# t-mat/lz4mt

Hardware: AMD Instinct MI355X
Metric: device-resident LZ4 GiB/s (compress, decompress) on 4 MiB blocks at 1/2/4/8 MI355X (higher is better)
Workload: dtype u8

## Files before the change

lz4mt_amd/csrc/lz4mt_kernels.hip:

```cpp
#include "lz4mt_device.h"
#include <stdio.h>
#include <string.h>

#include <algorithm>
#include <atomic>
#include <mutex>

#ifndef LZ4MT_PART
#define LZ4MT_PART 0
#endif

namespace lz4mt {

[[maybe_unused]] static bool link_cold() {
    const char* e = getenv("LZ4MT_AMD_BD_COLD");
    return e && e[0] == '1';
}

static void link_stats(const char* what, const uint32_t* changed, const uint32_t* firstU, int rounds,
                       uint32_t nBlocks, hipStream_t st) {
    const char* e = getenv("LZ4MT_AMD_BD_STATS");
    if (!e || e[0] != '1') return;
    uint32_t c[kLinkRounds + 1], f[kLinkRounds + 1];
    if (hipMemcpyAsync(c, changed, sizeof(c), hipMemcpyDeviceToHost, st) != hipSuccess ||
// ... 342 lines not shown
            int w;
            uint32_t ip = 0, cd = 0, maxb = 0, lim = 0, lit0 = 0;
            bool wasTest = false, early = false, beq = false;
            uint32_t eqb = 0;
            for (;;) {
                w = sm ? __ffsll((long long)sm) - 1 : 64;
                if (w == 64 || ((tmk >> w) & 1)) break;
                ip = rdlane(p, w);
                cd = rdlane(cand, w);
                wasTest = (ballot(isTest) >> w) & 1;
                {
                    const uint32_t lowL = !LINK ? 0u : (cd >= o0 ? lk.lowIn : lk.lowDict);
                    maxb = wasTest ? 0u : min(ip - anchor, cd > lowL ? cd - lowL : 0u);
                }
                lim = matchlimit - (ip + kMinMatch);
                V.cover(min(ip + kMinMatch + 256, n));
                const bool needV = (mm >> w) & 1;
                uint32_t vx = 0;
                if (needV && L == 0) vx = ld32u(s + cd) ^ rdlane(w0, w);
                beq = false;
                if (L + 1 <= maxb) beq = V.rd1(ip - L - 1) == V.rd1(cd - L - 1);
                eqb = 0;
                if (4 * L < lim) {
                    const uint32_t x = V.rd4(ip + kMinMatch + 4 * L) ^ V.rd4(cd + kMinMatch + 4 * L);
                    eqb = x ? ((uint32_t)__builtin_ctz(x) >> 3) : 4u;
                    eqb = min(eqb, lim - 4 * L);
                }
                STAMP_ADD(3, ts);
                if (ST) acc[12] += (mm >> w) & 1;
                lit0 = ip - anchor;
                early = lit0 <= 256 && op + 1 + ext_len(lit0) + lit0 + 64 <= O.flushed + kOutRing;
                if (early) stage_lits(V, O, anchor, 0, lit0, op + 1 + ext_len(lit0), false, 0);
                STAMP_ADD(4, ts);
                if (needV && (ballot(L == 0 && vx != 0) & 1)) {
                    if (ST) acc[11] += 1;
                    sm &= ~(1ull << w);
                    STAMP_ADD(5, ts);
                    continue;
                }
                if (ST) {
                    asm volatile("s_waitcnt vmcnt(0)" ::: "memory");
                }
                STAMP_ADD(5, ts);
                break;
            }
            const bool wTerm = (w < 64) && ((tmk >> w) & 1);
            const int wlim = (w == 64) ? 63 : (wTerm ? w - 1 : w);
            if (wlim >= 0 && live && (int)L <= wlim) {
                const uint64_t later = gmask & ~mask_le(L) & mask_le((uint32_t)wlim);
                if (!later) {
                    if (U16) T16[h] = (uint16_t)p;
                    else Traw[h] = TAG ? (p | (mytag << kPosBits)) : p;
                }
            }
            WAVE_SYNC();
            STAMP_ADD(6, ts);
            if (w == 64) {
                W.k0 += 64 - ns;
                W.hasIns = 0; W.hasTest = 0;
                continue;
            }
            if (wTerm) goto last_literals;

            uint32_t back = 0, mc = 0;
            bool backDone = maxb == 0, cntDone = false;
            for (;;) {
                if (!backDone) {
                    const uint64_t fm = ballot(!beq);
                    if (fm) { back += (uint32_t)(__ffsll((long long)fm) - 1); backDone = true; }
                    else { back += 64; backDone = back >= maxb; }
                }
                if (!cntDone) {
                    const uint64_t nf = ballot(eqb < 4);
                    if (nf) {
                        const int f = __ffsll((long long)nf) - 1;
                        mc += 4 * (uint32_t)f + rdlane(eqb, f);
                        cntDone = true;
                    } else {
                        mc += 256;
                    }
                }
                if (backDone && cntDone) break;
                beq = false;
                eqb = 0;
                const uint32_t kk = back + L + 1;
                if (!backDone && kk <= maxb) beq = V.rd1(ip - kk) == V.rd1(cd - kk);
                const uint32_t rel = mc + 4 * L;
                if (!cntDone && rel < lim) {
                    const uint32_t x = V.rd4(ip + kMinMatch + rel) ^ V.rd4(cd + kMinMatch + rel);
                    eqb = x ? ((uint32_t)__builtin_ctz(x) >> 3) : 4u;
                    eqb = min(eqb, lim - rel);
                }
            }
            STAMP_ADD(7, ts);
            const uint32_t mcf = mc + back;
            const uint32_t lit = lit0 - back;
            const uint32_t litExt = ext_len(lit);
            const uint32_t mlExt = ext_len(mcf);
            if (limited) {
                if (!wasTest && op + 1 + lit + 8 + lit / 255 > cap) return 0;
                if (op + 1 + litExt + lit + 2 + 6 + (mcf + 240) / 255 > cap) return 0;
            }
            const uint32_t litPos = op + 1 + litExt;
            if (!early || litExt != ext_len(lit0)) {
                put_head(O, op, lit, mcf < 15 ? mcf : 15);
                WAVE_SYNC();
                stage_lits(V, O, anchor, 0, lit, litPos, true, litPos);
            } else {
                put_head(O, op, lit, mcf < 15 ? mcf : 15);
            }
            {
                const uint32_t off = ip - cd, tpos = litPos + lit;
                O.flush_to(tpos);
                if (L < 2) O.put(tpos + L, L == 0 ? (off & 255) : (off >> 8));
                WAVE_SYNC();
                put_ext(O, tpos + 2, mlExt, mcf >= 15 ? (mcf - 15) % 255 : 0);
            }
            op = litPos + lit + 2 + mlExt;
            WAVE_SYNC();
            O.flush_to(op);
            STAMP_ADD(8, ts);
            const uint32_t ipe = ip + kMinMatch + mc;
            anchor = ipe;
            if (ipe >= mflimitP1) goto last_literals;
            W = Win{1, 1, ipe - 2, ipe, ipe + 1, 0};
        }
    }
last_literals : {
    const uint32_t run = n - anchor;
    if (limited && op + run + 1 + (run + 240) / 255 > cap) return 0;
    put_head(O, op, run, 0);
    const uint32_t litPos = op + 1 + ext_len(run);
    WAVE_SYNC();
    stage_lits(V, O, anchor, 0, run, litPos, true, litPos);
    op = litPos + run;
    O.finish(op);
}
    return (int32_t)op;
}

typedef const __attribute__((address_space(1))) uint32_t __attribute__((aligned(1))) g_cu32u;
typedef const __attribute__((address_space(1))) uint64_t __attribute__((aligned(1))) g_cu64u;
typedef __attribute__((address_space(3))) uint64_t __attribute__((aligned(1))) l_u64u;
typedef __attribute__((address_space(3))) uint32_t __attribute__((aligned(1))) l_u32u;
typedef __attribute__((address_space(3))) uint16_t __attribute__((aligned(1))) l_u16u;
typedef __attribute__((address_space(3))) uint64_t l_u64;

constexpr uint32_t kSR = 2048;
#ifndef LZ4MT_COUNT_LANES
#define LZ4MT_COUNT_LANES 32
#endif
constexpr uint32_t kCountLanes = LZ4MT_COUNT_LANES;
#ifndef LZ4MT_CATCH_LANES
#define LZ4MT_CATCH_LANES 64
#endif
constexpr uint32_t kCatchLanes = LZ4MT_CATCH_LANES;
static_assert(kCatchLanes >= 1 && kCatchLanes <= 64, "catch-up lanes");
constexpr uint64_t kCatchMask = kCatchLanes >= 64 ? ~0ull : (1ull << kCatchLanes) - 1ull;
static_assert(kCountLanes >= 1 && kCountLanes <= 63, "count lanes");
constexpr uint32_t kSRMirror = 64;
__device__ __forceinline__ void mskor2_rtn(l_u32* w16, uint32_t m16, uint32_t d16, l_u32* w8, uint32_t m8,
                                           uint32_t d8, uint32_t& o16, uint32_t& o8) {
    asm volatile("ds_mskor_rtn_b32 %0, %2, %3, %4\n\t"
                 "ds_mskor_rtn_b32 %1, %5, %6, %7\n\t"
                 "s_waitcnt lgkmcnt(0)"
                 : "=&v"(o16), "=&v"(o8)
                 : "v"((uint32_t)(uintptr_t)w16), "v"(m16), "v"(d16), "v"((uint32_t)(uintptr_t)w8), "v"(m8), "v"(d8)
                 : "memory");
}

__device__ __forceinline__ uint32_t gld4u(g_cu8* p) { return *(g_cu32u*)p; }
__device__ __forceinline__ uint64_t gld8u(g_cu8* p) { return *(g_cu64u*)p; }

struct SrcRing {
    g_cu8* s;
    uint32_t n;
    l_u8* r;
    uint32_t B;
    uint32_t pfPos;
    uint64_t pf;

    __device__ __forceinline__ uint64_t fetch(uint32_t c) const {
        const uint32_t pos = c + 8 * laneid();
        if (pos + 8 <= n) return gld8u(s + pos);
        uint64_t v = 0;
        for (uint32_t i = 0; i < 8; ++i)
            if (pos + i < n) v |= (uint64_t)s[pos + i] << (8 * i);
        return v;
    }
    __device__ __forceinline__ void store(uint32_t c, uint64_t v) {
        const uint32_t o = (c & (kSR - 1)) + 8 * laneid();
        *(l_u64*)(r + o) = v;
        if (o < kSRMirror) *(l_u64*)(r + kSR + o) = v;
    }
    __device__ __forceinline__ void init(uint32_t b0 = 0) {
        B = b0;
        for (uint32_t c = b0; c < b0 + kSR; c += 512) store(c, fetch(c));
        pfPos = b0 + kSR;
        pf = fetch(pfPos);
        WAVE_SYNC();
    }
    __device__ __forceinline__ void cover(uint32_t hi) {
        if (hi <= B + kSR) return;
        const uint32_t nb = (hi - kSR + 511) & ~511u;
        WAVE_SYNC();
        for (uint32_t c = (nb > B + kSR ? nb : B + kSR); c < nb + kSR; c += 512) store(c, c == pfPos ? pf : fetch(c));
        B = nb;
        pfPos = B + kSR;
        pf = fetch(pfPos);
        WAVE_SYNC();
    }
    __device__ __forceinline__ uint64_t rd8(uint32_t pos) const { return *(l_u64u*)(r + (pos & (kSR - 1))); }
};

__device__ __forceinline__ uint64_t bal(bool p) { return __builtin_amdgcn_ballot_w64(p); }
__device__ __forceinline__ uint32_t sff1(uint64_t m) { return m ? (uint32_t)__builtin_ctzll(m) : 64u; }
template <bool U16, bool SPLIT = false, bool LINK = false, bool P17 = false> struct V5Geo {
    static constexpr uint32_t kTE = U16 ? 8192u : 4096u;
    static constexpr uint32_t PB = P17 ? 17u : U16 ? 16u : (LINK ? kPosBits + 1 : kPosBits);
    static constexpr uint32_t PM = (1u << PB) - 1u;
    static constexpr bool SP = SPLIT || P17;
    static constexpr uint32_t TB = P17 ? 7u : SPLIT ? 8u : 32u - PB;
    static constexpr bool HT = !SP || U16;
    static __device__ __forceinline__ uint32_t tag(uint32_t w0) {
        if constexpr (HT && U16) return ((w0 * 2654435761u) >> (19 - TB)) & ((1u << TB) - 1u);
        else if constexpr (HT) return (uint32_t)(((uint64_t)w0 << 24) * 889523592379ull >> (52 - TB)) & ((1u << TB) - 1u);
        else return (w0 * 0x85EBCA77u) >> (32 - TB);
    }
    l_u32* T;
    __device__ __forceinline__ l_u16* T16() const { return (l_u16*)T; }
    __device__ __forceinline__ l_u8* TG() const { return (l_u8*)T + 2 * (kTE + 64); }
    __device__ __forceinline__ uint32_t ld(uint32_t i) const {
        return SP ? ((uint32_t)T16()[i] | ((uint32_t)TG()[i] << 16)) : T[i];
    }
    __device__ __forceinline__ void st(uint32_t i, uint32_t e) const {
        if (SP) { T16()[i] = (uint16_t)e; TG()[i] = (uint8_t)(e >> 16); } else T[i] = e;
    }
    __device__ __forceinline__ uint32_t rb(uint32_t i) const { return SP ? (uint32_t)T16()[i] : T[i]; }
    __device__ __forceinline__ uint32_t xchg(uint32_t i, uint32_t e) const {
        if constexpr (SP) {
            const uint32_t s16 = (i & 1u) * 16u, s8 = (i & 3u) * 8u;
            uint32_t o16, o8;
            mskor2_rtn((l_u32*)T16() + (i >> 1), 0xFFFFu << s16, (e & 0xFFFFu) << s16, (l_u32*)TG() + (i >> 2),
                       0xFFu << s8, ((e >> 16) & 0xFFu) << s8, o16, o8);
            return ((o16 >> s16) & 0xFFFFu) | (((o8 >> s8) & 0xFFu) << 16);
        } else {
            return __hip_atomic_exchange(T + i, e, __ATOMIC_RELAXED, __HIP_MEMORY_SCOPE_WAVEFRONT);
        }
    }
    static constexpr uint32_t kRbMask = SP ? 0xFFFFu : 0xFFFFFFFFu;
    __device__ __forceinline__ void sweep(uint32_t Tp) const {
        const uint32_t L = laneid();
        const uint32_t mk = (Tp + 65536u) & PM;
        for (uint32_t i = L; i < kTE; i += 64) {
            const uint32_t d = (Tp - ld(i)) & PM;
            if (d > 65536u && d <= 98304u) st(i, mk);
        }
        WAVE_SYNC();
    }
    __device__ __forceinline__ void init(uint32_t e0) const {
        const uint32_t L = laneid();
        if (SP) {
            const uint32_t p2 = (e0 & 0xFFFFu) * 0x10001u, t4 = (e0 >> 16) * 0x01010101u;
            for (uint32_t i = L; i < kTE / 8; i += 64) ((l_u4*)T16())[i] = (v4u){p2, p2, p2, p2};
            for (uint32_t i = L; i < kTE / 16; i += 64) ((l_u4*)TG())[i] = (v4u){t4, t4, t4, t4};
        } else {
            for (uint32_t i = L; i < kTE / 4; i += 64) ((l_u4*)T)[i] = (v4u){e0, e0, e0, e0};
        }
    }
};

struct PendSeq {
    uint32_t op, lit, mcf, off, anchor;
    uint32_t litExt, mlExt;
};
template <bool R8> struct SeqLayout {
    uint32_t total, a1, a2, token, litRem, mlRem, off;
    __device__ __forceinline__ explicit SeqLayout(const PendSeq& e) {
        a1 = 1 + e.litExt;
        a2 = a1 + e.lit;
        total = a2 + 2 + e.mlExt;
        token = ((e.lit < 15 ? e.lit : 15) << 4) | (e.mcf < 15 ? e.mcf : 15);
        if (R8) {
            litRem = e.lit + 240 + e.litExt;
            mlRem = e.mcf + 240 + e.mlExt;
        } else {
            litRem = e.lit + 240 - __umul24(255u, e.litExt);
            mlRem = e.mcf + 240 - __umul24(255u, e.mlExt);
        }
        off = e.off;
    }
};
template <bool R8>
__device__ __forceinline__ uint32_t pend_byte(const SeqLayout<R8>& e, uint32_t x, uint32_t litByte) {
    const uint32_t vM = x + 1 < e.total ? 255u : e.mlRem;
    const uint32_t vL = x + 1 < e.a1 ? 255u : e.litRem;
    const uint32_t vO = x == e.a2 ? e.off & 255u : e.off >> 8;
    uint32_t v = x < e.a2 + 2 ? vO : vM;
    v = x < e.a2 ? litByte : v;
    v = x < e.a1 ? vL : v;
    asm volatile("" : "+v"(v));
    return x == 0 ? e.token : v;
}
template <bool R8>
__device__ __forceinline__ void store_pend(const PendSeq& p, const SrcRing& V, g_cu8* __restrict__ s,
                                           g_u8* __restrict__ d) {
    const uint32_t L = laneid();
    PendSeq q = p;
    asm volatile("" : "+v"(q.lit), "+v"(q.mcf), "+v"(q.off), "+v"(q.litExt), "+v"(q.mlExt));
    const SeqLayout<R8> e(q);
    const uint32_t total = (uint32_t)__builtin_amdgcn_readfirstlane((int)e.total);
    if (p.anchor >= V.B && p.anchor + p.lit <= V.B + kSR) {
        uint32_t base = 0;
        do {
            const uint32_t x = min(base + L, e.total - 1);
            uint32_t lv = V.r[(p.anchor + x - e.a1) & (kSR - 1)];
            asm volatile("" : "+v"(lv));
            d[p.op + x] = (uint8_t)pend_byte(e, x, lv);
            base += 64;
        } while (base < total);
    } else {
        uint32_t base = 0;
        do {
            const uint32_t x = min(base + L, e.total - 1);
            uint32_t lv = s[(x >= e.a1 && x < e.a2) ? p.anchor + x - e.a1 : p.anchor];
            asm volatile("" : "+v"(lv));
            d[p.op + x] = (uint8_t)pend_byte(e, x, lv);
            base += 64;
        } while (base < total);
    }
}

constexpr uint32_t kPubShift = 16;
[[maybe_unused]] constexpr uint32_t kPubDone = 0x80000000u, kPubRaw = 0x40000000u, kPubLen = 0x3FFFFFFFu;
__device__ __forceinline__ void publish_progress(uint32_t* pub, uint32_t v) {
    asm volatile("s_waitcnt vmcnt(0)" ::: "memory");
    __builtin_amdgcn_fence(__ATOMIC_RELEASE, "agent");
    asm volatile("s_waitcnt vmcnt(0)" ::: "memory");
    if (laneid() == 0) __hip_atomic_store(pub, v, __ATOMIC_RELAXED, __HIP_MEMORY_SCOPE_AGENT);
}

constexpr uint32_t kWalkEnded = 0x80000000u;
__device__ __forceinline__ uint32_t walked_wait(uint32_t* ctl, uint32_t need) {
    const uint64_t t0 = __builtin_amdgcn_s_memrealtime();
    for (;;) {
        uint32_t v = 0;
        if (laneid() == 0) v = __hip_atomic_load(ctl, __ATOMIC_RELAXED, __HIP_MEMORY_SCOPE_AGENT);
        v = (uint32_t)__builtin_amdgcn_readfirstlane((int)v);
        if ((v & ~kWalkEnded) >= need || (v & kWalkEnded)) {
            __builtin_amdgcn_fence(__ATOMIC_ACQUIRE, "agent");
            asm volatile("s_waitcnt vmcnt(0)" ::: "memory");
            return v & ~kWalkEnded;
        }
        if (__builtin_amdgcn_s_memrealtime() - t0 > 3000000000ull) {
#if LZ4MT_WALK_DIAG
            if (laneid() == 0) {
                __hip_atomic_fetch_add(ctl + 5, 1u, __ATOMIC_RELAXED, __HIP_MEMORY_SCOPE_AGENT);
                __hip_atomic_store(ctl + 6, need, __ATOMIC_RELAXED, __HIP_MEMORY_SCOPE_AGENT);
                __hip_atomic_store(ctl + 7, v, __ATOMIC_RELAXED, __HIP_MEMORY_SCOPE_AGENT);
            }
#endif
            return 0;
        }
        __builtin_amdgcn_s_sleep(8);
    }
}
__device__ __forceinline__ void walk_publish(uint32_t* ctl, uint32_t v) {
    asm volatile("s_waitcnt vmcnt(0)" ::: "memory");
    (void)__hip_atomic_exchange(ctl, v, __ATOMIC_RELAXED, __HIP_MEMORY_SCOPE_AGENT);
}

constexpr uint32_t kPrioSimds = 8 * 8 * 2 * 16 * 4;
__device__ uint32_t g_simdFinish[kPrioSimds * 16];
struct SimdPrio {
    uint32_t base, slot;
    uint64_t t0;
    __device__ __forceinline__ void start() {
        const uint32_t hw = __builtin_amdgcn_s_getreg((31 << 11) | 4);
        const uint32_t xcc = __builtin_amdgcn_s_getreg((15 << 11) | 20);
        const uint32_t key = ((((xcc & 7) * 8 + ((hw >> 13) & 7)) * 2 + ((hw >> 12) & 1)) * 16 + ((hw >> 8) & 15)) * 4 +
                             ((hw >> 4) & 3);
        base = key * 16;
        slot = hw & 15;
        t0 = __builtin_amdgcn_s_memrealtime();
    }
    __device__ __forceinline__ void tick(uint32_t done, uint32_t total) const {
        const uint64_t now = __builtin_amdgcn_s_memrealtime();
        const float frac = (float)done / (float)total;
        const uint32_t fin = (uint32_t)t0 + (uint32_t)((float)(uint32_t)(now - t0) / (frac > 1e-3f ? frac : 1e-3f));
        const uint32_t L = laneid();
        if (L == 0) __hip_atomic_store(g_simdFinish + base + slot, fin, __ATOMIC_RELAXED, __HIP_MEMORY_SCOPE_AGENT);
#if LZ4MT_EXP_CUPRIO
        const uint32_t cb = base & ~63u;
        const uint32_t e = __hip_atomic_load(g_simdFinish + cb + L, __ATOMIC_RELAXED, __HIP_MEMORY_SCOPE_AGENT);
        const bool live = cb + L != base + slot && (int32_t)(e - (uint32_t)now) > 0;
        const uint32_t rank = (uint32_t)__builtin_popcountll(bal(live && (int32_t)(e - fin) < 0)) >> 1;
#else
        const uint32_t e = L < 16 ? __hip_atomic_load(g_simdFinish + base + L, __ATOMIC_RELAXED, __HIP_MEMORY_SCOPE_AGENT)
                                  : 0u;
        const bool live = L < 16 && L != slot && (int32_t)(e - (uint32_t)now) > 0;
        const uint32_t rank = (uint32_t)__builtin_popcountll(bal(live && (int32_t)(e - fin) < 0));
#endif
        if (rank >= 3) __builtin_amdgcn_s_setprio(3);
        else if (rank == 2) __builtin_amdgcn_s_setprio(2);
        else if (rank == 1) __builtin_amdgcn_s_setprio(1);
        else __builtin_amdgcn_s_setprio(0);
    }
    __device__ __forceinline__ void done() const {
        if (laneid() == 0) __hip_atomic_store(g_simdFinish + base + slot, 0u, __ATOMIC_RELAXED, __HIP_MEMORY_SCOPE_AGENT);
        __builtin_amdgcn_s_setprio(0);
    }
};
template <bool ST, bool U16, bool SPLIT = false, bool LINK = false, bool P17 = false, bool PUB = false,
          bool XH = false, bool XCHG = true, bool DUP = false>
__device__ int32_t encode_block_v5(g_cu8* __restrict__ s, uint32_t n, g_u8* __restrict__ d, uint32_t cap,
                                   l_u32* __restrict__ T, l_u8* __restrict__ R, uint64_t* acc,
                                   LinkArgs lk = LinkArgs{0, 0, 0, true}, uint32_t* pub = nullptr) {
    using G = V5Geo<U16, SPLIT, LINK, P17>;
    const G tab{T};
    const uint32_t L = laneid();
    uint64_t ts = STAMP_T();
    const uint32_t o0 = LINK ? kLinkO0 : 0u;
    auto xld4 = [&](uint32_t pos) -> uint32_t {
        if constexpr (!XH) {
            return gld4u(s + pos);
        } else {
            if (pos >= o0) return gld4u(s + pos);
            if (pos + 4 <= o0) return gld4u(s + pos + lk.shift);
            uint32_t v = 0;
            for (uint32_t j = 0; j < 4; ++j) {
                const uint32_t q = pos + j;
                v |= (uint32_t)s[q < o0 ? q + lk.shift : q] << (8 * j);
            }
            return v;
        }
    };
    auto xld1 = [&](uint32_t pos) -> uint32_t {
        if constexpr (!XH) return s[pos];
        else return s[pos < o0 ? pos + lk.shift : pos];
    };
    const uint32_t blen = n - o0;
    const uint32_t bound = blen + blen / 255 + 16;
    const bool limited = cap < bound;
    if (blen < (uint32_t)kMinLength) {
        if (limited && (LINK && blen == 0 ? cap == 0 : blen + 1 + (blen + 240) / 255 > cap)) return 0;
        if (L == 0) d[0] = (uint8_t)(blen << 4);
        for (uint32_t x = L; x < blen; x += 64) d[1 + x] = s[o0 + x];
        return (int32_t)(blen + 1);
    }
    if (!LINK || lk.fresh) {
        tab.init(o0 | (G::tag(gld4u(s + o0)) << G::PB));
    }
    if constexpr (XH) {
        if (!lk.fresh && lk.shift) {
            for (uint32_t i = L; i < G::kTE; i += 64) {
                const uint32_t e = tab.ld(i), pos = e & G::PM;
                if (pos != 0 && pos < o0) tab.st(i, pos | (G::tag(xld4(pos)) << G::PB));
            }
            WAVE_SYNC();
        }
    }
    SrcRing V{s, n, R, 0, 0, 0};
    V.init(o0);
#ifndef LZ4MT_NO_SIMD_PRIO
    constexpr bool kPrioT = !ST && !U16 && !SPLIT && !LINK && !P17 && !XH;
#else
    constexpr bool kPrioT = false;
#endif
    const bool prioOn = kPrioT && blen >= (1u << 20);
    SimdPrio prio{};
    uint32_t tickShift = 31;
    if (prioOn) {
        prio.start();
#ifndef LZ4MT_EXP_PRIO_SHIFT
#define LZ4MT_EXP_PRIO_SHIFT 7
#endif
        tickShift = (31 - __builtin_clz(blen)) - LZ4MT_EXP_PRIO_SHIFT;
    }
    const uint32_t capL = limited ? cap : 0xFFFFFFFFu;
    const uint32_t mflimitP1 = n - kMfLimit + 1;
    const uint32_t matchlimit = n - kLastLiterals;
    const uint32_t last4 = n - 4;
    const uint32_t dumIdx = G::kTE + L;
    uint32_t anchor = o0, op = 0;
    PendSeq pe{};
    bool havePe = false;
    bool done = false, fail = false;
    auto store_pending = [&]() {
#ifndef LZ4MT_EXP_R8ALL
        store_pend<U16 || P17>(pe, V, s, d);
#else
        store_pend<LZ4MT_EXP_R8ALL != 0>(pe, V, s, d);
#endif
        havePe = false;
    };
    uint32_t sBase = o0 + 1, k0 = 0, s0 = 1, j1 = 65, mode = 2;
    uint32_t spanHi = 61;
    uint32_t nextSweep = 32768;
#ifndef LZ4MT_FAST_WINDOW
#ifdef LZ4MT_NO_FAST_WINDOW
#define LZ4MT_FAST_WINDOW 0
#else
#define LZ4MT_FAST_WINDOW 15
#endif
#endif
    constexpr bool kFastT = (LZ4MT_FAST_WINDOW & 1) && !ST && !U16 && !SPLIT && !LINK && !P17 && !PUB && !XH && !DUP;
    constexpr bool kFastMargin = (LZ4MT_FAST_WINDOW & 2) != 0, kFastNoWide = (LZ4MT_FAST_WINDOW & 4) != 0;
    constexpr bool kFastFirst = (LZ4MT_FAST_WINDOW & 8) != 0;
    const uint32_t firstOff = L == 0 ? (uint32_t)-3 : (L == 1 ? (uint32_t)-1 : L - 2);
    constexpr uint32_t kFastSpanMax = 1016;
    constexpr uint32_t kFastEndGap = 1280;
    static_assert(kFastSpanMax + 17 + 4 + 4 * kCountLanes + 8 + kMfLimit + 64 <= kFastEndGap, "fast phase end distance");
    constexpr uint32_t kFastOutSlack = 64;
    const uint32_t fastEndV = n > o0 + kFastEndGap ? n - kFastEndGap : 0u;
    uint32_t fastEndS = (!kFastMargin || !limited) ? fastEndV : 0u;
    for (;;) {
#define V5_FAST false
#include "lz4mt_v5_window.inc"
#undef V5_FAST
        if constexpr (kFastT) {
            if (done) break;
#define V5_FAST true
#include "lz4mt_v5_window.inc"
#undef V5_FAST
            done = fail || anchor >= mflimitP1;
        } else {
            break;
        }
    }
    if (prioOn) prio.done();
    if (fail) return 0;
    if (havePe) store_pending();
    {
        const uint32_t run = n - anchor;
        if (limited && op + run + 1 + (run + 240) / 255 > cap) return 0;
        const uint32_t ext = ext_len(run), rem = run >= 15 ? (run - 15) % 255 : 0u;
        if (L == 0) d[op] = (uint8_t)((run < 15 ? run : 15) << 4);
        for (uint32_t x = L; x < ext; x += 64) d[op + 1 + x] = (uint8_t)(x + 1 < ext ? 255u : rem);
        op += 1 + ext;
        for (uint32_t x = L; x < run; x += 64) d[op + x] = s[anchor + x];
        op += run;
    }
    return (int32_t)op;
}

#define ENCODE_LDS                                                     \
    __shared__ __attribute__((aligned(16))) uint32_t ELDS[5120];       \
    uint32_t* const T = ELDS;                                          \
    uint8_t* const S = (uint8_t*)(ELDS + 4096);                        \
    uint32_t* const X = ELDS + 4352;
static_assert(kSR + kSRMirror <= 3072, "ring exceeds the shared scratch");
static_assert(kDedup == 1024, "scratch layout");

#if LZ4MT_PART != 2
#if LZ4MT_EXP_BLKTIME
constexpr uint32_t kExpBlkMax = 16384;
__device__ uint64_t g_expBlk[3 * kExpBlkMax];
#endif
template <bool XC>
__global__ void __launch_bounds__(64) k_encode(const uint8_t* __restrict__ src, uint64_t srcSize, uint32_t blockSize,
                                               uint8_t* __restrict__ slots, uint64_t slotStride,
                                               uint32_t capOverride, int32_t* __restrict__ csize) {
    ENCODE_LDS
    const uint32_t b = blockIdx.x;
    const uint64_t off = (uint64_t)b * blockSize;
    const uint32_t n = (uint32_t)((srcSize - off) < blockSize ? (srcSize - off) : blockSize);
    const uint32_t cap = (capOverride == 0xFFFFFFFFu) ? n : capOverride;
    g_cu8* s = gptr(src) + off;
    g_u8* d = gptr(slots) + (uint64_t)b * slotStride;
    l_u32* Tl = (l_u32*)T;
    l_u8* Sl = (l_u8*)S;
    l_u8* Xl = (l_u8*)X;
#if LZ4MT_EXP_BLKTIME
    const uint64_t t0 = wall_clock64();
#endif
    int32_t r;
    if (n < (uint32_t)kLimit64K)
        r = encode_block<true, false, false>(s, n, d, cap, Tl, Sl, (l_u32*)Xl, Xl + kRingE, nullptr);
    else if (n <= (1u << kPosBits))
        [[clang::always_inline]] r =
            encode_block_v5<false, false, false, false, false, false, false, XC>(s, n, d, cap, Tl, Xl, nullptr);
    else
        r = encode_block<false, false, false>(s, n, d, cap, Tl, Sl, (l_u32*)Xl, Xl + kRingE, nullptr);
    if (laneid() == 0) csize[b] = r;
#if LZ4MT_EXP_BLKTIME
    if (laneid() == 0 && b < kExpBlkMax) {
        g_expBlk[3 * b] = t0;
        g_expBlk[3 * b + 1] = wall_clock64();
        g_expBlk[3 * b + 2] = ((uint64_t)__builtin_amdgcn_s_getreg((15 << 11) | 20) << 32) |
                              (uint64_t)__builtin_amdgcn_s_getreg((31 << 11) | 4);
    }
#endif
}
#if LZ4MT_EXP_BLKTIME
extern "C" int lz4mtHipExpBlockTimes(uint64_t* out, uint32_t nb) {
    if (nb > kExpBlkMax) nb = kExpBlkMax;
    return hipMemcpyFromSymbol(out, HIP_SYMBOL(g_expBlk), (size_t)nb * 24) == hipSuccess ? (int)nb : -1;
}
#endif

template <bool XC>
__global__ void __launch_bounds__(64) k_encode_pub(const uint8_t* __restrict__ src, uint64_t srcSize,
                                                   uint32_t blockSize, uint8_t* __restrict__ slots,
                                                   uint64_t slotStride, int32_t* __restrict__ csize,
                                                   uint32_t* __restrict__ pub) {
    ENCODE_LDS
    const uint32_t b = blockIdx.x;
    const uint64_t off = (uint64_t)b * blockSize;
    const uint32_t n = (uint32_t)((srcSize - off) < blockSize ? (srcSize - off) : blockSize);
    g_cu8* s = gptr(src) + off;
    g_u8* d = gptr(slots) + (uint64_t)b * slotStride;
    l_u32* Tl = (l_u32*)T;
    l_u8* Sl = (l_u8*)S;
    l_u8* Xl = (l_u8*)X;
    int32_t r;
    if (n < (uint32_t)kLimit64K)
        r = encode_block<true, false, false>(s, n, d, n, Tl, Sl, (l_u32*)Xl, Xl + kRingE, nullptr);
    else if (n <= (1u << kPosBits))
        r = encode_block_v5<false, false, false, false, false, true, false, XC>(s, n, d, n, Tl, Xl, nullptr,
                                                                                LinkArgs{0, 0, 0, true}, pub + b);
    else
        r = encode_block<false, false, false>(s, n, d, n, Tl, Sl, (l_u32*)Xl, Xl + kRingE, nullptr);
    if (laneid() == 0) csize[b] = r;
    publish_progress(pub + b, kPubDone | (r > 0 ? (uint32_t)r : kPubRaw));
}

__global__ void __launch_bounds__(64) k_xchg_order(uint32_t* ok) {
    __shared__ uint32_t W[64];
    const uint32_t L = laneid();
    bool good = true;
    for (uint32_t pat = 0; pat < 3; ++pat) {
        W[L] = 0xFFFF0000u | L;
        WAVE_SYNC();
        const uint32_t a = pat == 0 ? 0u : pat == 1 ? (L & 3u) : (L * 37u) % 7u;
        const uint32_t got = __hip_atomic_exchange((l_u32*)W + a, L, __ATOMIC_RELAXED, __HIP_MEMORY_SCOPE_WAVEFRONT);
        WAVE_SYNC();
        uint32_t want = 0xFFFF0000u | a, last = 64;
        for (uint32_t j = 0; j < 64; ++j) {
            const uint32_t aj = pat == 0 ? 0u : pat == 1 ? (j & 3u) : (j * 37u) % 7u;
            if (aj == a && j < L) want = j;
            if (aj == L) last = j;
        }
        good = good && got == want && (last == 64 || W[L] == last);
        WAVE_SYNC();
    }
    for (uint32_t fb = 16; fb >= 8; fb -= 8) {
        const uint32_t nf = 32u / fb, fm = (1u << fb) - 1u;
        W[L] = 0xA5A5A5A5u ^ L;
        WAVE_SYNC();
        const uint32_t sel = (L * 5u) % (4u * nf), a = sel / nf, sh = (sel % nf) * fb;
        uint32_t o16, o8;
        mskor2_rtn((l_u32*)W + a, fm << sh, ((L + 1u) & fm) << sh, (l_u32*)W + 63, 0u, 0u, o16, o8);
        WAVE_SYNC();
        uint32_t want = ((0xA5A5A5A5u ^ a) >> sh) & fm, fin = 0xA5A5A5A5u ^ L;
        for (uint32_t j = 0; j < 64; ++j) {
            const uint32_t sj = (j * 5u) % (4u * nf), shj = (sj % nf) * fb;
            if (sj == sel && j < L) want = (j + 1u) & fm;
            if (sj / nf == L) fin = (fin & ~(fm << shj)) | (((j + 1u) & fm) << shj);
        }
        good = good && ((o16 >> sh) & fm) == want && (L >= 4 || W[L] == fin);
        WAVE_SYNC();
    }
    const bool all = __builtin_amdgcn_ballot_w64(!good) == 0;
    if (L == 0) *ok = all ? 1u : 0u;
}

static std::atomic<int> g_xchg_state[64];
static bool probe_forced_readback() {
    const char* e = getenv("LZ4MT_AMD_ENC_PROBE");
    return e && !strcmp(e, "readback");
}
static hipError_t xchg_check(int dev) {
    static std::mutex mu;
    std::lock_guard<std::mutex> g(mu);
    if (g_xchg_state[dev].load()) return hipSuccess;
    hipStream_t ps = nullptr;
    uint32_t* d = nullptr;
    uint32_t h = 0;
    hipError_t e = hipStreamCreateWithFlags(&ps, hipStreamNonBlocking);
    if (e == hipSuccess) e = hipMalloc(&d, 4);
    if (e == hipSuccess) {
        hipLaunchKernelGGL(k_xchg_order, dim3(1), dim3(64), 0, ps, d);
        e = hipGetLastError();
    }
    if (e == hipSuccess) e = hipMemcpyAsync(&h, d, 4, hipMemcpyDeviceToHost, ps);
    if (e == hipSuccess) e = hipStreamSynchronize(ps);
    if (d) (void)hipFree(d);
    if (ps) (void)hipStreamDestroy(ps);
    if (e != hipSuccess) return e;
    g_xchg_state[dev].store(h == 1 ? 1 : -1, std::memory_order_release);
    if (h != 1)
        fprintf(stderr, "lz4mt_amd: device %d does not apply a wave's same-address LDS exchanges in lane order; "
                        "the block encoders use the read-back table probe there\n", dev);
    return hipSuccess;
}
hipError_t encoder_path(hipStream_t st, bool* xc) {
    *xc = false;
    int dev = 0;
    if (hipGetDevice(&dev) != hipSuccess || dev < 0 || dev >= 64) return hipErrorInvalidDevice;
    if (probe_forced_readback()) return hipSuccess;
    int v = g_xchg_state[dev].load(std::memory_order_acquire);
    if (v == 0) {
        hipStreamCaptureStatus cs = hipStreamCaptureStatusNone;
        if (st && hipStreamIsCapturing(st, &cs) == hipSuccess && cs != hipStreamCaptureStatusNone) return hipSuccess;
        if (const hipError_t e = xchg_check(dev); e != hipSuccess) return e;
        v = g_xchg_state[dev].load(std::memory_order_acquire);
    }
    *xc = v > 0;
    return hipSuccess;
}
hipError_t encoder_ready(hipStream_t st) {
    bool xc = false;
    if (const hipError_t e = encoder_path(st, &xc); e != hipSuccess) return e;
    return xc ? hipSuccess : hipErrorNotSupported;
}

extern "C" int lz4mtHipCheckEncoderOrder(void) {
    int n = 0, dev = 0;
    if (hipGetDeviceCount(&n) != hipSuccess || n <= 0 || hipGetDevice(&dev) != hipSuccess || dev < 0 || dev >= 64)
        return -1;
    if (g_xchg_state[dev].load() == 0 && xchg_check(dev) != hipSuccess) return -1;
    return g_xchg_state[dev].load() > 0 ? 1 : 0;
}

extern "C" int lz4mtHipEncoderProbe(void) {
    int n = 0;
    if (hipGetDeviceCount(&n) != hipSuccess || n <= 0) return -1;
    bool xc = false;
    if (encoder_path(nullptr, &xc) != hipSuccess) return -1;
    return xc ? 1 : 0;
}

hipError_t launch_encode_pub(const uint8_t* src, uint64_t srcSize, uint32_t blockSize, uint32_t nBlocks,
                             uint8_t* slots, int32_t* csize, uint32_t* pub, hipStream_t st) {
    bool xc = true;
    if (const hipError_t r = encoder_path(st, &xc); r != hipSuccess) return r;
    if (nBlocks == 0) return hipSuccess;
    hipLaunchKernelGGL(xc ? k_encode_pub<true> : k_encode_pub<false>, dim3(nBlocks), dim3(64), 0, st, src, srcSize,
                       blockSize, slots, (uint64_t)blockSize, csize, pub);
    return hipGetLastError();
}

template <bool XC>
__global__ void __launch_bounds__(64) k_encode_p17(const uint8_t* __restrict__ src, uint64_t srcSize,
                                                   uint32_t blockSize, uint8_t* __restrict__ slots,
                                                   uint64_t slotStride, uint32_t capOverride,
                                                   int32_t* __restrict__ csize) {
    __shared__ __attribute__((aligned(16))) uint32_t PLDS[(2 * (4096 + 64) + (4096 + 64) + kSR + kSRMirror) / 4];
    const uint32_t b = blockIdx.x;
    const uint64_t off = (uint64_t)b * blockSize;
    const uint32_t n = (uint32_t)((srcSize - off) < blockSize ? (srcSize - off) : blockSize);
    if (n < (uint32_t)kLimit64K || n > (1u << kPosBits)) return;
    const uint32_t cap = (capOverride == 0xFFFFFFFFu) ? n : capOverride;
    l_u8* Xl = (l_u8*)PLDS + 3 * (4096 + 64);
    int32_t r;
    [[clang::always_inline]] r = encode_block_v5<false, false, false, false, true, false, false, XC>(
        gptr(src) + off, n, gptr(slots) + (uint64_t)b * slotStride, cap, (l_u32*)PLDS, Xl, nullptr);
    if (laneid() == 0) csize[b] = r;
}

__global__ void __launch_bounds__(64) k_encode_stats(const uint8_t* __restrict__ src, uint64_t srcSize,
                                                     uint32_t blockSize, uint8_t* __restrict__ slots,
                                                     uint64_t slotStride, int32_t* __restrict__ csize,
                                                     uint64_t* __restrict__ stats) {
    ENCODE_LDS
    const uint32_t b = blockIdx.x;
    const uint64_t off = (uint64_t)b * blockSize;
    const uint32_t n = (uint32_t)((srcSize - off) < blockSize ? (srcSize - off) : blockSize);
    uint64_t acc[16] = {0};
    int32_t r;
    g_cu8* s = gptr(src) + off;
    g_u8* d = gptr(slots) + b * slotStride;
    l_u8* Xl = (l_u8*)X;
    if (n < (uint32_t)kLimit64K)
        r = encode_block<true, false, true>(s, n, d, n, (l_u32*)T, (l_u8*)S, (l_u32*)Xl, Xl + kRingE, acc);
    else if (n <= (1u << kPosBits))
        r = encode_block_v5<true, false>(s, n, d, n, (l_u32*)T, Xl, acc);
    else
        r = encode_block<false, false, true>(s, n, d, n, (l_u32*)T, (l_u8*)S, (l_u32*)Xl, Xl + kRingE, acc);
    if (laneid() == 0) {
        csize[b] = r;
        for (int i = 0; i < 16; ++i) stats[b * 16 + i] = acc[i];
    }
}

constexpr uint32_t kE16TabWords = (8192 + 64) * 3 / 4;
constexpr uint32_t kE16Words = kE16TabWords + (kSR + kSRMirror) / 4;
template <bool XC>
__global__ void __launch_bounds__(64) k_encode16(const uint8_t* __restrict__ src, uint64_t srcSize,
                                                 uint32_t blockSize, uint8_t* __restrict__ slots,
                                                 uint64_t slotStride, uint32_t capOverride,
                                                 int32_t* __restrict__ csize) {
    __shared__ uint32_t E16[kE16Words];
    const uint32_t b = blockIdx.x;
    const uint64_t off = (uint64_t)b * blockSize;
    const uint32_t n = (uint32_t)((srcSize - off) < blockSize ? (srcSize - off) : blockSize);
    const uint32_t cap = (capOverride == 0xFFFFFFFFu) ? n : capOverride;
    const int32_t r = encode_block_v5<false, true, true, false, false, false, false, XC>(
        gptr(src) + off, n, gptr(slots) + (uint64_t)b * slotStride, cap, (l_u32*)E16, (l_u8*)(E16 + kE16TabWords),
        nullptr);
    if (laneid() == 0) csize[b] = r;
}

struct BatchChunk {
    g_cu8* s;
    g_u8* d;
    uint32_t n, cap;
    bool bad;
};
__device__ __forceinline__ BatchChunk batch_chunk(const uint8_t* const* __restrict__ srcPtrs,
                                                  const uint32_t* __restrict__ srcSizes, uint32_t maxChunk,
                                                  uint8_t* const* __restrict__ dstPtrs,
// ... 2697 lines not shown
```

lz4mt_amd/csrc/lz4mt_v5_window.inc:

```
{
    constexpr bool FAST = V5_FAST;
    constexpr bool FIRST = FAST && kFastFirst;
    bool sw = false;
    bool fcont = false;
    while (!done && !sw) {
      uint32_t w, ip, cd, maxb, cw, iw, bi, bc;
      bool wTerm;
      do {
        if (ST) acc[10] += 1;
        if (P17) {
            while (sBase >= nextSweep) {
                tab.sweep(nextSweep);
                nextSweep += 32768;
            }
        }
        const uint32_t j = L - 2;
        const int32_t jx = (int32_t)j - (int32_t)j1;
        uint32_t p = sBase + __umul24(j, s0) + (uint32_t)max(jx, 0);
        const uint32_t step = FIRST ? 1u : s0 + (jx >= 0 ? 1u : 0u);
        const uint32_t sHi = sBase + (FIRST ? 61u : spanHi);
        const bool insOn = FIRST ? true : mode != 0;
        const uint32_t insPos = !FIRST && mode == 2 ? o0 : sBase - 3, testPos = sBase - 1;
        p = L == 0 ? insPos : (L == 1 ? testPos : p);
        if constexpr (FIRST) p = sBase + firstOff;
        const uint64_t roleM = FIRST ? 3ull : (uint64_t)((0x130u >> (4 * mode)) & 3u);
        const uint64_t liveM = FAST ? ~3ull | roleM : (bal(p <= mflimitP1) & ~3ull) | roleM;
        const uint64_t tmk = FAST ? 0ull : bal(p + step > mflimitP1) & liveM & ~3ull;
        const bool live = FIRST ? true : __builtin_amdgcn_inverse_ballot_w64(liveM);
        const bool term = FAST ? false : __builtin_amdgcn_inverse_ballot_w64(tmk);
        const uint32_t lo = insOn ? insPos : sBase;
        const uint32_t hi = (FAST || sHi < mflimitP1 ? sHi : mflimitP1) + 8;
        uint64_t v8;
        const bool wide = FAST && kFastNoWide ? false : hi - lo > 1024;
        if constexpr (kPrioT) {
            if (!wide && hi > V.B + kSR) {
                const uint32_t oldB = V.B;
                V.cover(hi);
                if (prioOn && ((oldB ^ V.B) >> tickShift)) prio.tick(V.B - o0, blen);
            }
        } else {
            if (!wide) V.cover(hi);
        }
        v8 = V.rd8(p);
        if (wide) {
            if (ST) acc[13] += 1;
            v8 = gld8u(s + (p < n - 8 ? p : n - 8));
            uint32_t a = (uint32_t)v8, b = (uint32_t)(v8 >> 32);
            asm volatile("" : "+v"(a), "+v"(b));
            v8 = ((uint64_t)b << 32) | a;
        }
        const uint32_t w0 = (uint32_t)v8;
        uint32_t h, tg;
        if constexpr (G::HT && U16) {
            const uint32_t P = w0 * 2654435761u;
            h = P >> 19;
            tg = (P >> (19 - G::TB)) & ((1u << G::TB) - 1u);
        } else if constexpr (G::HT) {
            const uint64_t P = (v8 << 24) * 889523592379ull;
            h = (uint32_t)(P >> 52);
            tg = (uint32_t)(P >> (52 - G::TB)) & ((1u << G::TB) - 1u);
        } else {
            h = lz4_hash<U16>(w0, (uint32_t)(v8 >> 32));
            tg = G::tag(w0);
        }
        const uint32_t mark = (P17 ? p & G::PM : p) | (tg << G::PB);
        const uint32_t ti = live ? h : dumIdx;
        uint32_t told;
        uint64_t pend = 0;
        if constexpr (XCHG) {
            told = tab.xchg(ti, mark);
        } else {
            told = tab.ld(ti);
            tab.st(ti, mark);
            WAVE_SYNC();
            const uint32_t sv = tab.rb(ti);
            pend = bal(sv != (mark & G::kRbMask));
        }
        const uint32_t dq = (p - told) & G::PM;
        uint32_t cand = P17 ? p - dq : told & G::PM;
        const uint64_t cokM = bal((P17 ? dq <= kDistMax : cand + kDistMax >= p) && (!LINK || cand >= lk.candLow)) &
                              liveM & ~tmk & ~1ull;
        uint64_t mm = cokM & bal((told >> G::PB) == (mark >> G::PB));
        bool maybe = __builtin_amdgcn_inverse_ballot_w64(mm);
        uint64_t sm = mm | tmk;
        STAMP_ADD(0, ts);
        w = 64;
        bool dd = false, twDone = false, twRedo = false;
        uint64_t gmask, aliased = 0;
        auto table_writes = [&](uint32_t ws, bool wsTerm, uint32_t pB) {
            const int wlim = (ws == 64) ? 63 : (wsTerm ? (int)ws - 1 : (int)ws);
            const bool le = (int)L <= wlim;
            if constexpr (XCHG) {
                if (twRedo) (void)tab.xchg((live && le) ? h : dumIdx, mark);
                const bool first = P17 ? dq >= p - pB : (told & G::PM) <= pB;
                tab.st(((FAST || live) && !le && first) ? h : dumIdx, told);
            } else {
                tab.st(((FAST || live) && !le) ? h : dumIdx, told);
                if (pend || twRedo) {
                    const uint64_t upto = wlim < 0 ? 0ull : mask_le((uint32_t)wlim);
                    const bool lastM = !dd || !(gmask & ~mask_le(L) & upto);
                    tab.st((live && le && lastM) ? h : dumIdx, mark);
                }
            }
            WAVE_SYNC();
        };
        bool again = true;
        while (again) {
            w = sff1(sm);
            if (!dd && (pend & mask_le(w < 63 ? w : 63))) {
                if (ST) acc[12] += 1;
                dd = true;
                int pred = -1;
                gmask = 1ull << L;
                uint64_t todo = pend;
                while (todo) {
                    const uint32_t key = rdlane(h, (int)sff1(todo));
                    const uint64_t m = bal(live && h == key);
                    const bool inG = (m >> L) & 1;
                    const uint64_t below = m & ((1ull << L) - 1ull);
                    pred = inG ? (below ? 63 - __clzll((long long)below) : -1) : pred;
                    gmask = inG ? m : gmask;
                    todo &= ~m;
                }
                const int pi = (pred < 0 ? 0 : pred) * 4;
                const uint32_t pw = (uint32_t)__builtin_amdgcn_ds_bpermute(pi, (int)w0);
                const uint32_t pp = (uint32_t)__builtin_amdgcn_ds_bpermute(pi, (int)p);
                const bool ok = live && L != 0 && !term && pred >= 0 && pp + kDistMax >= p && pw == w0 &&
                                (!LINK || pp >= lk.candLow);
                maybe = maybe && pred < 0;
                cand = pred >= 0 ? pp : cand;
                mm = bal(maybe);
                sm = (bal(ok) | mm | tmk) & ~aliased;
            } else {
                wTerm = w < 64 && ((tmk >> w) & 1);
                again = false;
                if (w < 64 && !wTerm) {
                    ip = rdlane(p, (int)w);
                    cd = rdlane(cand, (int)w);
                    {
                        const uint32_t lowL = !LINK ? 0u : (cd >= o0 ? lk.lowIn : lk.lowDict);
                        maxb = w == 1 ? 0u : min(ip - anchor, cd > lowL ? cd - lowL : 0u);
                    }
                    const bool cOn = L <= kCountLanes;
                    const uint32_t ci = cOn ? cd + 4 * L : cd, ii = cOn ? ip + 4 * L : ip;
                    const bool bOn = L < maxb && L < kCatchLanes;
                    cw = xld4(FAST || ci < last4 ? ci : last4);
                    iw = gld4u(s + (FAST || ii < last4 ? ii : last4));
                    uint32_t bix = bOn ? ip - L - 1 : o0, bcx = bOn ? cd - L - 1 : o0;
                    asm volatile("" : "+v"(bix), "+v"(bcx));
                    bi = s[bix];
                    bc = xld1(bcx);
                    if (havePe) store_pending();
                    table_writes(w, false, ip);
                    twDone = true;
                    if (((mm >> w) & 1) && rdlane(cw, 0) != rdlane(w0, (int)w)) {
                        if (ST) acc[11] += 1;
                        __builtin_amdgcn_s_waitcnt(0x0F70);
                        aliased |= 1ull << w;
                        sm &= ~(1ull << w);
                        again = true;
                        twDone = false;
                        twRedo = true;
                    }
                }
            }
        }
        if (havePe) store_pending();
        if (!twDone && (!XCHG || w < 64 || twRedo)) table_writes(w, wTerm, rdlane(p, (int)(w < 64 ? w - 1 : 63)));
        STAMP_ADD(1, ts);
        STAMP_ADD(2, ts);
        if constexpr (FIRST) {
            if (w == 64) {
                sBase += 62;
                fcont = true;
                sw = true;
            }
        } else if (w == 64) {
            sBase += 62 * s0 + (62 > j1 ? 62 - j1 : 0u);
            k0 += 62;
            s0 = (63 + k0) >> 6;
            j1 = (k0 < 65 ? 65u : ((k0 - 1) & ~63u) + 65) - k0;
            mode = 0;
            spanHi = 61 * s0 + (61 > j1 ? 61 - j1 : 0u);
            if constexpr (FAST) sw = spanHi > kFastSpanMax || sBase > fastEndS;
        }
      } while (!FIRST && w == 64 && !(FAST && sw));
        if (FAST && w == 64) {
        } else if (wTerm) {
            done = true;
        } else {
            asm volatile("" ::"v"(bi), "v"(bc));
            uint64_t fm = ~(bal(L < maxb) & bal(bi == bc)) & kCatchMask;
            uint32_t back = 0;
            if (kCatchLanes < 64 && fm == 0) {
                back = kCatchLanes;
                const uint32_t kb = back + L + 1;
                const bool on = kb <= maxb;
                fm = ~bal(on && s[on ? ip - kb : o0] == xld1(on ? cd - kb : o0));
            }
            while (fm == 0 && back + 64 < maxb) {
                back += 64;
                const uint32_t kb = back + L + 1;
                const bool on = kb <= maxb;
                fm = ~bal(on && s[on ? ip - kb : o0] == xld1(on ? cd - kb : o0));
            }
            back = fm ? back + (uint32_t)__builtin_ctzll(fm) : maxb;
            const uint32_t lim = matchlimit - (ip + kMinMatch);
            uint32_t mc;
            {
                const uint32_t rel = 4 * L - 4;
                const uint32_t x = cw ^ iw;
                uint32_t e = x ? ((uint32_t)__builtin_ctz(x) >> 3) : 4u;
                if constexpr (!FAST) {
                    e = min(e, lim - rel);
                    e = rel < lim ? e : 0u;
                }
                const uint64_t nf = bal(e < 4) & (mask_le(kCountLanes) & ~1ull);
                if (nf) {
                    const uint32_t f = (uint32_t)__builtin_ctzll(nf);
                    mc = 4 * (f - 1) + rdlane(e, (int)f);
                } else {
                    mc = 4 * kCountLanes;
                    uint64_t nf2 = 0;
                    while (!nf2) {
                        const uint32_t r2 = mc + 4 * L;
                        const uint32_t a2 = ip + kMinMatch + r2, c2 = cd + kMinMatch + r2;
                        const uint32_t x2 = gld4u(s + (a2 < last4 ? a2 : last4)) ^ xld4(c2 < last4 ? c2 : last4);
                        uint32_t e2 = min(x2 ? ((uint32_t)__builtin_ctz(x2) >> 3) : 4u, lim - r2);
                        e2 = r2 < lim ? e2 : 0u;
                        nf2 = bal(e2 < 4);
                        mc += nf2 ? 4 * (uint32_t)__builtin_ctzll(nf2) + rdlane(e2, (int)__builtin_ctzll(nf2))
                                  : 256u;
                    }
                }
            }
            STAMP_ADD(3, ts);
            const uint32_t lit = ip - anchor - back, mcf = mc + back;
            pe.lit = lit;
            pe.mcf = mcf;
            pe.off = ip - cd;
            pe.anchor = anchor;
            {
                const uint32_t litExt = ext_len(lit), mlExt = ext_len(mcf);
                pe.litExt = litExt;
                pe.mlExt = mlExt;
                if constexpr (!(FAST && kFastMargin)) {
                    if (op + 2 * (lit + mcf) + 16 > capL) {
                        fail = (w != 1 && op + 1 + lit + 8 + lit / 255 > cap) ||
                               (op + 1 + litExt + lit + 2 + 6 + (mcf + 240) / 255 > cap);
                    }
                }
                pe.op = op;
                havePe = FAST && kFastMargin ? true : !fail;
                if constexpr (PUB) {
                    if ((op ^ (op + 1 + litExt + lit + 2 + mlExt)) >> kPubShift) publish_progress(pub, op);
                }
                op += 1 + litExt + lit + 2 + mlExt;
            }
            const uint32_t ipe = ip + kMinMatch + mc;
            anchor = ipe;
            if constexpr (FAST) {
                if constexpr (kFastMargin) sw = ipe >= fastEndS;
                else sw = fail || ipe >= fastEndS;
            } else {
                done = fail || ipe >= mflimitP1;
                if constexpr (kFastT) {
                    if (kFastMargin && fastEndS == 0 && op + (n - ipe) + (n - ipe) / 255 + kFastOutSlack <= cap)
                        fastEndS = fastEndV;
                    sw = !fail && ipe < fastEndS;
                }
            }
            sBase = ipe + 1;
            if constexpr (!FIRST) {
                mode = 1;
                k0 = 0;
                s0 = 1;
                j1 = 65;
                spanHi = 61;
            }
            STAMP_ADD(4, ts);
        }
    }
    if constexpr (FIRST) {
        k0 = fcont ? 62u : 0u;
        j1 = fcont ? 3u : 65u;
        mode = fcont ? 0u : 1u;
        spanHi = fcont ? 119u : 61u;
        s0 = 1;
    }
}
```

Baseline: 51.12.

## Fold backward catch-up into forward word compare lanes in fast window

In the fast first-window path, the backward match extension now reuses the same 4-byte word load and compare as the forward count. Extra lanes load words at negative offsets and use leading-zero counts. This replaces the separate byte-wise catch-up loads and ballots, and caps backward extension at w-1 bytes. A relaxed ring-buffer check is also enabled for pending sequence stores. The fast phase additionally requires a minimum start distance so the backward word loads stay in bounds. Capping backward extension to about 64 bytes may slightly change compression output.

```diff
diff --git a/lz4mt_amd/csrc/lz4mt_kernels.hip b/lz4mt_amd/csrc/lz4mt_kernels.hip
--- a/lz4mt_amd/csrc/lz4mt_kernels.hip
+++ b/lz4mt_amd/csrc/lz4mt_kernels.hip
@@ -668,15 +668,20 @@
     asm volatile("" : "+v"(v));
     return x == 0 ? e.token : v;
 }
-template <bool R8>
+constexpr int kPendRingLo = 1, kPendNoBytes = 4;
+template <bool R8, int FS = 0>
 __device__ __forceinline__ void store_pend(const PendSeq& p, const SrcRing& V, g_cu8* __restrict__ s,
                                            g_u8* __restrict__ d) {
+    if constexpr ((FS & kPendNoBytes) != 0) return;
     const uint32_t L = laneid();
+#define LZ4MT_PEND_IN_RING \
+    ((FS & kPendRingLo) ? p.anchor >= V.B : p.anchor >= V.B && p.anchor + p.lit <= V.B + kSR)
     PendSeq q = p;
     asm volatile("" : "+v"(q.lit), "+v"(q.mcf), "+v"(q.off), "+v"(q.litExt), "+v"(q.mlExt));
     const SeqLayout<R8> e(q);
     const uint32_t total = (uint32_t)__builtin_amdgcn_readfirstlane((int)e.total);
-    if (p.anchor >= V.B && p.anchor + p.lit <= V.B + kSR) {
+    if (LZ4MT_PEND_IN_RING) {
+#undef LZ4MT_PEND_IN_RING
         uint32_t base = 0;
         do {
             const uint32_t x = min(base + L, e.total - 1);
@@ -867,13 +872,37 @@
 #ifdef LZ4MT_NO_FAST_WINDOW
 #define LZ4MT_FAST_WINDOW 0
 #else
-#define LZ4MT_FAST_WINDOW 15
+#define LZ4MT_FAST_WINDOW 63
 #endif
 #endif
     constexpr bool kFastT = (LZ4MT_FAST_WINDOW & 1) && !ST && !U16 && !SPLIT && !LINK && !P17 && !PUB && !XH && !DUP;
     constexpr bool kFastMargin = (LZ4MT_FAST_WINDOW & 2) != 0, kFastNoWide = (LZ4MT_FAST_WINDOW & 4) != 0;
     constexpr bool kFastFirst = (LZ4MT_FAST_WINDOW & 8) != 0;
+    constexpr bool kFastCatchW = kFastFirst && (LZ4MT_FAST_WINDOW & 16) != 0;
+    [[maybe_unused]] constexpr bool kFastRingLo = kFastFirst && kFastNoWide && (LZ4MT_FAST_WINDOW & 32) != 0;
+#ifdef LZ4MT_EXP_NO_PEND_BYTES
+    constexpr int kFastStoreFS = kPendNoBytes;
+#else
+    constexpr int kFastStoreFS = kFastRingLo ? kPendRingLo : 0;
+#endif
+#ifndef LZ4MT_EXP_R8ALL
+    [[maybe_unused]] constexpr bool kPendR8 = U16 || P17;
+#else
+    [[maybe_unused]] constexpr bool kPendR8 = LZ4MT_EXP_R8ALL != 0;
+#endif
     const uint32_t firstOff = L == 0 ? (uint32_t)-3 : (L == 1 ? (uint32_t)-1 : L - 2);
+    constexpr uint32_t kCatchWords = 16;
+#ifndef LZ4MT_CATCH_GATE
+#define LZ4MT_CATCH_GATE 1
+#endif
+    [[maybe_unused]] constexpr bool kCatchGate = LZ4MT_CATCH_GATE != 0;
+    static_assert(kCountLanes + 1 + kCatchWords <= 64, "catch-up word lanes");
+    [[maybe_unused]] constexpr uint64_t kBackLanes = ((1ull << kCatchWords) - 1ull) << (kCountLanes + 1);
+    uint32_t rtOff = 0;
+    if constexpr (kFastCatchW && kFastT)
+        rtOff = L <= kCountLanes ? 4 * L : (L <= kCountLanes + kCatchWords ? 4 * kCountLanes - 4 * L : 0u);
+    constexpr uint32_t kFastBeg = kDistMax + 1 + 4 * kCatchWords;
+    [[maybe_unused]] const uint32_t fastBegS = o0 + kFastBeg;
     constexpr uint32_t kFastSpanMax = 1016;
     constexpr uint32_t kFastEndGap = 1280;
     static_assert(kFastSpanMax + 17 + 4 + 4 * kCountLanes + 8 + kMfLimit + 64 <= kFastEndGap, "fast phase end distance");
diff --git a/lz4mt_amd/csrc/lz4mt_v5_window.inc b/lz4mt_amd/csrc/lz4mt_v5_window.inc
--- a/lz4mt_amd/csrc/lz4mt_v5_window.inc
+++ b/lz4mt_amd/csrc/lz4mt_v5_window.inc
@@ -1,6 +1,8 @@
 {
     constexpr bool FAST = V5_FAST;
     constexpr bool FIRST = FAST && kFastFirst;
+    constexpr bool CW = FAST && kFastCatchW;
+    constexpr bool STF = FIRST && kFastStoreFS != 0;
     bool sw = false;
     bool fcont = false;
     while (!done && !sw) {
@@ -137,10 +139,18 @@
                 if (w < 64 && !wTerm) {
                     ip = rdlane(p, (int)w);
                     cd = rdlane(cand, (int)w);
-                    {
+                    if constexpr (CW) {
+                        maxb = w - 1;
+                    } else {
                         const uint32_t lowL = !LINK ? 0u : (cd >= o0 ? lk.lowIn : lk.lowDict);
                         maxb = w == 1 ? 0u : min(ip - anchor, cd > lowL ? cd - lowL : 0u);
                     }
+                    if constexpr (CW) {
+                        const uint32_t ro =
+                            !kCatchGate || (int32_t)rtOff >= -(int32_t)((maxb + 3) & ~3u) ? rtOff : 0u;
+                        cw = xld4(cd + ro);
+                        iw = gld4u(s + (ip + ro));
+                    } else {
                     const bool cOn = L <= kCountLanes;
                     const uint32_t ci = cOn ? cd + 4 * L : cd, ii = cOn ? ip + 4 * L : ip;
                     const bool bOn = L < maxb && L < kCatchLanes;
@@ -150,7 +160,15 @@
                     asm volatile("" : "+v"(bix), "+v"(bcx));
                     bi = s[bix];
                     bc = xld1(bcx);
-                    if (havePe) store_pending();
+                    }
+                    if (havePe) {
+                        if constexpr (STF) {
+                            store_pend<kPendR8, kFastStoreFS>(pe, V, s, d);
+                            havePe = false;
+                        } else {
+                            store_pending();
+                        }
+                    }
                     table_writes(w, false, ip);
                     twDone = true;
                     if (((mm >> w) & 1) && rdlane(cw, 0) != rdlane(w0, (int)w)) {
@@ -165,7 +183,14 @@
                 }
             }
         }
-        if (havePe) store_pending();
+        if (havePe) {
+            if constexpr (STF) {
+                store_pend<kPendR8, kFastStoreFS>(pe, V, s, d);
+                havePe = false;
+            } else {
+                store_pending();
+            }
+        }
         if (!twDone && (!XCHG || w < 64 || twRedo)) table_writes(w, wTerm, rdlane(p, (int)(w < 64 ? w - 1 : 63)));
         STAMP_ADD(1, ts);
         STAMP_ADD(2, ts);
@@ -189,9 +214,11 @@
         } else if (wTerm) {
             done = true;
         } else {
+            uint64_t fm = 0;
+            uint32_t back = 0;
+            if constexpr (!CW) {
             asm volatile("" ::"v"(bi), "v"(bc));
-            uint64_t fm = ~(bal(L < maxb) & bal(bi == bc)) & kCatchMask;
-            uint32_t back = 0;
+            fm = ~(bal(L < maxb) & bal(bi == bc)) & kCatchMask;
             if (kCatchLanes < 64 && fm == 0) {
                 back = kCatchLanes;
                 const uint32_t kb = back + L + 1;
@@ -205,17 +232,34 @@
                 fm = ~bal(on && s[on ? ip - kb : o0] == xld1(on ? cd - kb : o0));
             }
             back = fm ? back + (uint32_t)__builtin_ctzll(fm) : maxb;
+            }
             const uint32_t lim = matchlimit - (ip + kMinMatch);
             uint32_t mc;
             {
                 const uint32_t rel = 4 * L - 4;
                 const uint32_t x = cw ^ iw;
-                uint32_t e = x ? ((uint32_t)__builtin_ctz(x) >> 3) : 4u;
+                uint32_t e;
+                if constexpr (CW) {
+                    const bool bk = __builtin_amdgcn_inverse_ballot_w64(kBackLanes);
+                    e = x ? ((bk ? (uint32_t)__builtin_clz(x) : (uint32_t)__builtin_ctz(x)) >> 3) : 4u;
+                } else {
+                    e = x ? ((uint32_t)__builtin_ctz(x) >> 3) : 4u;
+                }
                 if constexpr (!FAST) {
                     e = min(e, lim - rel);
                     e = rel < lim ? e : 0u;
                 }
-                const uint64_t nf = bal(e < 4) & (mask_le(kCountLanes) & ~1ull);
+                const uint64_t nfAll = bal(e < 4);
+                const uint64_t nf = nfAll & (mask_le(kCountLanes) & ~1ull);
+                if constexpr (CW) {
+                    const uint64_t nb = nfAll & kBackLanes;
+                    if (nb) {
+                        const uint32_t f = (uint32_t)__builtin_ctzll(nb);
+                        back = min(4 * (f - (kCountLanes + 1)) + rdlane(e, (int)f), maxb);
+                    } else {
+                        back = maxb;
+                    }
+                }
                 if (nf) {
                     const uint32_t f = (uint32_t)__builtin_ctzll(nf);
                     mc = 4 * (f - 1) + rdlane(e, (int)f);
@@ -268,6 +312,7 @@
                     if (kFastMargin && fastEndS == 0 && op + (n - ipe) + (n - ipe) / 255 + kFastOutSlack <= cap)
                         fastEndS = fastEndV;
                     sw = !fail && ipe < fastEndS;
+                    if constexpr (kFastCatchW) sw = sw && ipe >= fastBegS;
                 }
             }
             sBase = ipe + 1;
```

Measured after the change: 55.31 (median of 6 runs). +8.2%, better.
